# sebrahimi1988/dss-ml-at-scale

Hardware: NVIDIA H100
Metric: series fitted+forecast/sec (higher is better)
Workload: dtype f32

## Files before the change

dss-ml-at-scale_b200/csrc/fit_tc.cu:

```cuda
#include "mmf_internal.cuh"
#include "sm90_ptx.cuh"

namespace mmf {
namespace {

using namespace sm90;

constexpr int TILE_M = 128;
constexpr int KC = 32;
constexpr int NGROUPS = 2;
constexpr int FOLD_CHUNKS = 18;
constexpr int MAX_PRED = 64;
constexpr int BULK_MAX_PRED = 28;
constexpr int Y_STAGE_BYTES = TILE_M * KC * 4;
constexpr int AT_STAGE_BYTES = 2 * P * KC * 4;
constexpr int THREADS = 416;
constexpr int TILE_RING = 4;
constexpr int WARP_EPI0 = 8, WARP_PROD = 12;

template <int STAGES, int OBUF, bool SE = false>
struct SmemLayoutT {
  static constexpr int y = 0;
  static constexpr int at = y + STAGES * Y_STAGE_BYTES;
  static constexpr int apred = at + STAGES * AT_STAGE_BYTES;
  static constexpr int ostage = apred + MAX_PRED * P * 4;
  static constexpr int acc = ostage + OBUF * TILE_M * BULK_MAX_PRED * 4;
  static constexpr int nm = acc + 2 * NGROUPS * TILE_M * P * 4;
  static constexpr int cc = nm + 2 * NGROUPS * TILE_M * 2;
  static constexpr int tiles = cc + 2 * TILE_M * 4;
  static constexpr int bars = tiles + TILE_RING * 4;
  static constexpr int n_bars = 2 * STAGES + 6 + 2 * TILE_RING;
  static constexpr int ss = bars + n_bars * 8;
  static constexpr int sfac = ss + (SE ? 2 * NGROUPS * TILE_M * 8 : 0);
  static constexpr int total = sfac + (SE ? MAX_PRED * 4 : 0);
  static_assert(total + 1024 <= 232448, "exceeds the 227 KB of shared memory a CTA can opt into");
};

__device__ __forceinline__ float dot16(const float* __restrict__ arow, const float (&g)[P], float s) {
  const float4* ap = reinterpret_cast<const float4*>(arow);
  const float4 a0 = ap[0], a1 = ap[1], a2 = ap[2], a3 = ap[3];
  s = fmaf(a0.x, g[0], s);  s = fmaf(a0.y, g[1], s);  s = fmaf(a0.z, g[2], s);  s = fmaf(a0.w, g[3], s);
  s = fmaf(a1.x, g[4], s);  s = fmaf(a1.y, g[5], s);  s = fmaf(a1.z, g[6], s);  s = fmaf(a1.w, g[7], s);
  s = fmaf(a2.x, g[8], s);  s = fmaf(a2.y, g[9], s);  s = fmaf(a2.z, g[10], s); s = fmaf(a2.w, g[11], s);
  s = fmaf(a3.x, g[12], s); s = fmaf(a3.y, g[13], s); s = fmaf(a3.z, g[14], s); s = fmaf(a3.w, g[15], s);
  return s;
}

__device__ __forceinline__ bool is_finite_bits(float x) { return (__float_as_uint(x) & 0x7f800000u) != 0x7f800000u; }

__device__ __forceinline__ float centring_constant(const float4& a, const float4& b, int t_fit) {
  const float v[8] = {a.x, a.y, a.z, a.w, b.x, b.y, b.z, b.w};
  float c = t_fit > 7 ? v[7] : __int_as_float(0x7fc00000);
#pragma unroll
  for (int i = 6; i >= 0; --i) c = (i < t_fit && is_finite_bits(v[i])) ? v[i] : c;
  return c;
}

__device__ __forceinline__ void bt_write_moments(const BtArgs& bt, int k, int grp, int64_t n, const TileRec& tr, int frow0,
                                                 int t4, const float (&acc)[2][P], bool folded, const float* sacc) {
#pragma unroll
  for (int h = 0; h < 2; ++h)
#pragma unroll
    for (int j = 0; j < 2; ++j) {
      const int rt = 64 * h + frow0 + 8 * j;
      if (rt >= tr.nrows) continue;
      float* __restrict__ dst = bt.mom + (((int64_t)k * 2 + grp) * n + tr.row0 + rt) * P + 2 * t4;
#pragma unroll
      for (int i = 0; i < 2; ++i) {
        const int q = 4 * i + 2 * j;
        float2 v = make_float2(acc[h][q] + acc[h][q + P / 2], acc[h][q + 1] + acc[h][q + 1 + P / 2]);
        if (folded) {
          const float2 o = *reinterpret_cast<const float2*>(sacc + rt * P + 8 * i + 2 * t4);
          v.x = o.x + v.x; v.y = o.y + v.y;
        }
        *reinterpret_cast<float2*>(dst + 8 * i) = v;
      }
    }
}

__device__ __forceinline__ float lds32(uint32_t addr) {
  float v;
  asm volatile("ld.shared.f32 %0, [%1];" : "=f"(v) : "r"(addr));
  return v;
}

template <int STAGES, int OBUF, bool MULTI, bool SE = false, bool BT = false>
__global__ void __launch_bounds__(THREADS, 1)
fit_tc_kernel(const __grid_constant__ TcLaunch tl, const DesignView d, const FitArgs a,
              uint32_t* __restrict__ pending_count, const int n_tiles, const int n_chunks, const MultiView mv,
              const SeArgs se, const BtArgs bt) {
  static_assert(!SE || !MULTI, "standard errors are built for the single-calendar launch");
  static_assert(!BT || !(MULTI || SE), "backtests are built for the single-calendar launch");
  using SmemLayout = SmemLayoutT<STAGES, OBUF, SE>;
  auto tile_rec = [&](int ti) -> TileRec {
    if (MULTI) {
      if (ti >= n_tiles) return TileRec{0, 0, 0, 1};
      const int4 v = __ldg(reinterpret_cast<const int4*>(mv.tiles) + ti);
      return TileRec{v.x, v.y, v.z, v.w};
    }
    const int64_t left = a.n - (int64_t)ti * TILE_M;
    return TileRec{ti * TILE_M, (int)(left >= TILE_M ? TILE_M : (left > 0 ? left : 0)), 0, n_chunks};
  };
  extern __shared__ unsigned char smem_dyn[];
  unsigned char* smem = reinterpret_cast<unsigned char*>((reinterpret_cast<uintptr_t>(smem_dyn) + 1023) & ~uintptr_t(1023));
  const uint32_t sbase = smem_u32(smem);
  const uint32_t s_y = sbase + SmemLayout::y;
  const uint32_t s_at = sbase + SmemLayout::at;
  float* s_apred = reinterpret_cast<float*>(smem + SmemLayout::apred);
  float* s_ostage = reinterpret_cast<float*>(smem + SmemLayout::ostage);
  float* s_acc = reinterpret_cast<float*>(smem + SmemLayout::acc);
  uint16_t* s_nm = reinterpret_cast<uint16_t*>(smem + SmemLayout::nm);
  float* s_cc = reinterpret_cast<float*>(smem + SmemLayout::cc);
  double* s_ss = reinterpret_cast<double*>(smem + SmemLayout::ss);
  float* s_sfac = reinterpret_cast<float*>(smem + SmemLayout::sfac);
#ifdef MMF_TC_NO_COLLECT
  const bool collect = false;
#else
  const bool collect = a.recs != nullptr && d.t_fit <= 65535;
#endif
  const uint32_t s_bars = sbase + SmemLayout::bars;
  const int warp = threadIdx.x >> 5;
  const int lane = threadIdx.x & 31;
  auto bar_full = [&](int s) { return s_bars + 8u * s; };
  auto bar_empty = [&](int s) { return s_bars + 8u * (STAGES + s); };
  auto bar_accfull = [&](int b) { return s_bars + 8u * (2 * STAGES + b); };
  auto bar_accempty = [&](int b) { return s_bars + 8u * (2 * STAGES + 2 + b); };
  auto bar_cc = [&](int b) { return s_bars + 8u * (2 * STAGES + 4 + b); };
  auto bar_tfull = [&](int s) { return s_bars + 8u * (2 * STAGES + 6 + s); };
  auto bar_tempty = [&](int s) { return s_bars + 8u * (2 * STAGES + 6 + TILE_RING + s); };
  int* s_tiles = reinterpret_cast<int*>(smem + SmemLayout::tiles);
  auto take_tile = [&](int lt) -> int {
    const int sl = lt % TILE_RING;
    mbar_wait(bar_tfull(sl), (lt / TILE_RING) & 1);
    const int t = *reinterpret_cast<volatile int*>(s_tiles + sl);
    __syncwarp();
    if (lane == 0) mbar_arrive(bar_tempty(sl));
    return t;
  };

  if (blockIdx.x == 0 && threadIdx.x == 0 && a.zero_next != nullptr) {
#pragma unroll
    for (int i = 0; i < CTR_WORDS; ++i) a.zero_next[i] = 0u;
  }
  if (warp == WARP_PROD) {
    if (lane == 0) {
      for (int s = 0; s < STAGES; ++s) {
        mbar_init(bar_full(s), 1);
        mbar_init(bar_empty(s), 4);
      }
      for (int b = 0; b < 2; ++b) {
        mbar_init(bar_accfull(b), NGROUPS * 128);
        mbar_init(bar_accempty(b), 4);
        mbar_init(bar_cc(b), 128);
      }
      for (int sl = 0; sl < TILE_RING; ++sl) {
        mbar_init(bar_tfull(sl), 1);
        mbar_init(bar_tempty(sl), NGROUPS * 4 + 4);
      }
      fence_mbar_init();
      prefetch_tensormap(tl.tmap_y);
      prefetch_tensormap(tl.tmap_at);
    }
  } else if (warp >= WARP_EPI0) {
    if (!a.skip_pred && !MULTI)
      for (int i = threadIdx.x - WARP_EPI0 * 32; i < a.n_pred * P; i += 128)
        s_apred[i] = __ldg(d.apred + (size_t)a.pred_start * P + i);
    if (SE && !a.skip_pred)
      for (int i = threadIdx.x - WARP_EPI0 * 32; i < a.n_pred; i += 128) s_sfac[i] = __ldg(se.sfac + a.pred_start + i);
  }
  __syncthreads();
  if (threadIdx.x == 0) pdl_launch_dependents();

  if (warp == WARP_PROD) {
    int stage = 0;
    uint32_t phase = 0;
    int last_cal = -1;
    uint32_t* claim_ctr = pending_count + CTR_TILE_CLAIM;
    int tile = blockIdx.x;
    for (int lt = 0;; ++lt) {
      const int sl = lt % TILE_RING;
      mbar_wait(bar_tempty(sl), ((lt / TILE_RING) & 1) ^ 1u);
      const bool more = tile < n_tiles;
      uint32_t claim = 0;
      if (lane == 0) {
        if (more) claim = atomicAdd(claim_ctr, 1u);
        s_tiles[sl] = more ? tile : -1;
        mbar_arrive(bar_tfull(sl));
      }
      __syncwarp();
      if (!more) break;
      const TileRec tr = tile_rec(tile);
      const void* tmy = MULTI ? static_cast<const void*>(mv.tmaps_y + (size_t)tr.cal * 128) : static_cast<const void*>(tl.tmap_y);
      if (MULTI && tr.cal != last_cal) { fence_tensormap_acquire(tmy); last_cal = tr.cal; }
      const int at_row = MULTI ? tr.cal * 2 * P : 0;
      for (int ch = 0; ch < tr.n_chunks; ++ch) {
        mbar_wait(bar_empty(stage), phase ^ 1u);
        tma_load_2d_x2_elect(bar_full(stage), Y_STAGE_BYTES + AT_STAGE_BYTES,
                             s_y + stage * Y_STAGE_BYTES, tmy, ch * KC, tr.row0, L2_EVICT_NORMAL,
                             s_at + stage * AT_STAGE_BYTES, tl.tmap_at, ch * KC, at_row,
                             MULTI ? L2_EVICT_NORMAL : L2_EVICT_LAST);
        if (++stage == STAGES) { stage = 0; phase ^= 1u; }
      }
      tile = static_cast<int>(gridDim.x + __shfl_sync(0xffffffffu, claim, 0));
    }
  } else if (warp < NGROUPS * 4) {
    const int grp = warp >> 2;
    const int r = threadIdx.x & 127;
    const uint32_t row_off = static_cast<uint32_t>(r) * 128u;
    const uint32_t sw = static_cast<uint32_t>(r & 7);
    const int g8 = lane >> 2, t4 = lane & 3;
    const int frow0 = 16 * (warp & 3) + g8;
    uint32_t gc = 0;
    for (int lt = 0;; ++lt) {
      const int tile = take_tile(lt);
      if (tile < 0) break;
      const TileRec tr = tile_rec(tile);
      bool bad = false;
      float cf[2][2];
      float acc[2][P];
#pragma unroll
      for (int h = 0; h < 2; ++h)
#pragma unroll
        for (int i = 0; i < P; ++i) acc[h][i] = 0.f;
      const bool scan = collect && (!MULTI || r < tr.nrows);
      const int seg = (grp ^ (int)gc) & 1;
      int nm = 0;
      unsigned long long packq = 0ull;
      const int ab = lt & 1;
      float* __restrict__ sacc = s_acc + (ab * NGROUPS + grp) * TILE_M * P;
      auto sacc_at = [&](int h, int j, int i) {
        return reinterpret_cast<float2*>(sacc + (64 * h + frow0 + 8 * j) * P + 8 * i + 2 * t4);
      };
      bool folded = false;
      int since_fold = 0;
      double ssq[2][2] = {{0.0, 0.0}, {0.0, 0.0}};
      for (int ch = seg; ch < tr.n_chunks; ch += NGROUPS) {
        const uint32_t k = gc + static_cast<uint32_t>(ch);
        const int stage = static_cast<int>(k % STAGES);
        mbar_wait(bar_full(stage), (k / STAGES) & 1u);
        const uint32_t sy = s_y + stage * Y_STAGE_BYTES;
        if (ch == seg) {
          if (seg == 0) {
            mbar_wait(bar_accempty(ab), ((lt >> 1) & 1) ^ 1u);
            float c = 0.f;
            if (d.has_constant && r < tr.nrows) {
              const uint32_t rowp = sy + row_off;
              c = centring_constant(lds128(rowp + (sw << 4)), lds128(rowp + ((1u ^ sw) << 4)), MULTI ? KC : d.t_fit);
            }
            bad = collect && !is_finite_bits(c);
            s_cc[ab * TILE_M + r] = bad ? 0.f : c;
            mbar_arrive(bar_cc(ab));
          }
          mbar_wait(bar_cc(ab), (lt >> 1) & 1);
#pragma unroll
          for (int h = 0; h < 2; ++h)
#pragma unroll
            for (int j = 0; j < 2; ++j) cf[h][j] = s_cc[ab * TILE_M + 64 * h + frow0 + 8 * j];
        }
        if (scan) {
          const uint32_t rowp = sy + row_off;
          float4 v[8];
#pragma unroll
          for (int q = 0; q < 8; ++q) v[q] = lds128(rowp + ((static_cast<uint32_t>(q) ^ sw) << 4));
          float chk = 0.f;
#pragma unroll
          for (int q = 0; q < 8; ++q) {
            chk = fmaf(v[q].x, 0.f, chk); chk = fmaf(v[q].y, 0.f, chk);
            chk = fmaf(v[q].z, 0.f, chk); chk = fmaf(v[q].w, 0.f, chk);
          }
          if (!(chk == 0.f)) {
            unsigned gaps = 0u;
#pragma unroll
            for (int q = 0; q < 8; ++q)
              gaps |= (is_finite_bits(v[q].x) ? 0u : 1u << (4 * q)) | (is_finite_bits(v[q].y) ? 0u : 2u << (4 * q)) |
                      (is_finite_bits(v[q].z) ? 0u : 4u << (4 * q)) | (is_finite_bits(v[q].w) ? 0u : 8u << (4 * q));
            uint16_t* __restrict__ mt = a.recs[(int64_t)tr.row0 + r].miss_t + seg * SOLVE_SEG;
            const int tbase = ch * KC;
            while (gaps) {
              const int pos = __ffs(gaps) - 1;
              gaps &= gaps - 1u;
              packq = (packq >> 16) | (static_cast<unsigned long long>(tbase + pos) << 48);
              ++nm;
              if ((nm & 3) == 0 && nm <= SOLVE_SEG) *reinterpret_cast<unsigned long long*>(mt + nm - 4) = packq;
              if constexpr (BT) if (nm == SOLVE_SEG + 1)
                reinterpret_cast<uint16_t*>(&a.recs[(int64_t)tr.row0 + r].ss)[seg] = static_cast<uint16_t>(tbase + pos);
            }
          }
        }
        uint32_t ahi[2][KC / 8][4], alo[2][KC / 8][4];
        const int lim = d.t_fit - ch * KC;
#pragma unroll
        for (int h = 0; h < 2; ++h)
#pragma unroll
          for (int j = 0; j < 2; ++j) {
            const uint32_t rowp = sy + static_cast<uint32_t>(64 * h + frow0 + 8 * j) * 128u + t4 * 4;
            float part = 0.f;
#pragma unroll
            for (int kk = 0; kk < KC / 8; ++kk)
#pragma unroll
              for (int hf = 0; hf < 2; ++hf) {
                float x = lds32(rowp + ((static_cast<uint32_t>(2 * kk + hf) ^ static_cast<uint32_t>(g8)) << 4));
                if (collect) x = is_finite_bits(x) ? x : cf[h][j];
                const float rr = x - cf[h][j];
                const uint32_t hb = __float_as_uint(rr) & 0xFFFFE000u;
                ahi[h][kk][j + 2 * hf] = hb;
                alo[h][kk][j + 2 * hf] = __float_as_uint(rr - __uint_as_float(hb));
                if (SE) {
                  const float rs = 4 * (2 * kk + hf) + t4 < lim ? rr : 0.f;
                  part = fmaf(rs, rs, part);
                }
              }
            if (SE) ssq[h][j] += static_cast<double>(part);
          }
        const uint64_t bdesc0 = gmma_desc_k_sw128(s_at + stage * AT_STAGE_BYTES);
        uint32_t bt_in = 0;
        if constexpr (BT) {
          const int s0 = ch * KC;
          uint32_t pre = 0;
#pragma unroll
          for (int k = 0; k < MMF_BT_MAX_ORIGINS - 1; ++k) {
            pre |= (bt.t_orig[k] >= s0 - KC && bt.t_orig[k] <= s0 ? 1u : 0u) << k;
            bt_in |= (bt.t_orig[k] > s0 && bt.t_orig[k] < s0 + KC ? 1u : 0u) << k;
          }
          while (pre) {
            const int k = __ffs(pre) - 1;
            pre &= pre - 1u;
            bt_write_moments(bt, k, grp, a.n, tr, frow0, t4, acc, folded, sacc);
          }
        }
        if constexpr (BT) {
        if (bt_in != 0u) {
          int lo = 0;
          uint32_t m = bt_in;
          for (;;) {
            const int k = m ? __ffs(m) - 1 : -1;
            const int hi = k >= 0 ? __ldg(&bt.cals[k].t_fit) - ch * KC : KC;
            wgmma_fence();
#pragma unroll
            for (int h = 0; h < 2; ++h)
#pragma unroll
              for (int kk = 0; kk < KC / 8; ++kk) {
                const uint64_t bdesc = bdesc0 + static_cast<uint64_t>(kk * 2);
                uint32_t fh[4], fl[4];
#pragma unroll
                for (int e = 0; e < 4; ++e) {
                  const int col = 8 * kk + 4 * (e >> 1) + t4;
                  const bool in = col >= lo && col < hi;
                  fh[e] = in ? ahi[h][kk][e] : 0u;
                  fl[e] = in ? alo[h][kk][e] : 0u;
                }
                wgmma_m64n32k8_tf32_rs(acc[h], fh, bdesc);
#ifndef MMF_TC_NO_LO_TERM
                wgmma_m64n32k8_tf32_rs(acc[h], fl, bdesc);
#endif
              }
            wgmma_commit();
            wgmma_wait<0>();
            wgmma_fence_regs(acc[0]);
            wgmma_fence_regs(acc[1]);
            if (k < 0) break;
            bt_write_moments(bt, k, grp, a.n, tr, frow0, t4, acc, folded, sacc);
            m &= m - 1u;
            lo = hi;
          }
        } else {
        wgmma_fence();
#pragma unroll
        for (int h = 0; h < 2; ++h)
#pragma unroll
          for (int kk = 0; kk < KC / 8; ++kk) {
            const uint64_t bdesc = bdesc0 + static_cast<uint64_t>(kk * 2);
            wgmma_m64n32k8_tf32_rs(acc[h], ahi[h][kk], bdesc);
#ifndef MMF_TC_NO_LO_TERM
            wgmma_m64n32k8_tf32_rs(acc[h], alo[h][kk], bdesc);
#endif
          }
        wgmma_commit();
        wgmma_wait<0>();
        wgmma_fence_regs(acc[0]);
        wgmma_fence_regs(acc[1]);
        }
        } else {
        wgmma_fence();
#pragma unroll
        for (int h = 0; h < 2; ++h)
#pragma unroll
          for (int kk = 0; kk < KC / 8; ++kk) {
            const uint64_t bdesc = bdesc0 + static_cast<uint64_t>(kk * 2);
            wgmma_m64n32k8_tf32_rs(acc[h], ahi[h][kk], bdesc);
#ifndef MMF_TC_NO_LO_TERM
            wgmma_m64n32k8_tf32_rs(acc[h], alo[h][kk], bdesc);
#endif
          }
        wgmma_commit();
        wgmma_wait<0>();
        wgmma_fence_regs(acc[0]);
        wgmma_fence_regs(acc[1]);
        }
        __syncwarp();
        if (lane == 0) mbar_arrive(bar_empty(stage));
        if (++since_fold == FOLD_CHUNKS && ch + NGROUPS < tr.n_chunks) {
          if (!folded) mbar_wait(bar_accempty(ab), ((lt >> 1) & 1) ^ 1u);
#pragma unroll
          for (int h = 0; h < 2; ++h)
#pragma unroll
            for (int j = 0; j < 2; ++j)
#pragma unroll
              for (int i = 0; i < 2; ++i) {
                const int q = 4 * i + 2 * j;
                float2 f = make_float2(acc[h][q] + acc[h][q + P / 2], acc[h][q + 1] + acc[h][q + 1 + P / 2]);
                if (folded) { const float2 o = *sacc_at(h, j, i); f.x = o.x + f.x; f.y = o.y + f.y; }
                *sacc_at(h, j, i) = f;
              }
#pragma unroll
          for (int h = 0; h < 2; ++h)
#pragma unroll
            for (int i = 0; i < P; ++i) acc[h][i] = 0.f;
          folded = true;
          since_fold = 0;
        }
      }
      if (scan && (nm & 3) != 0 && nm < SOLVE_SEG) {
        uint16_t* __restrict__ mt = a.recs[(int64_t)tr.row0 + r].miss_t + seg * SOLVE_SEG;
        *reinterpret_cast<unsigned long long*>(mt + (nm & ~3)) = packq >> (16 * (4 - (nm & 3)));
      }
      if constexpr (BT) {
        const int s_end = ((tr.n_chunks - 1 - seg) / NGROUPS * NGROUPS + seg + 1) * KC;
        uint32_t rest = 0;
#pragma unroll
        for (int k = 0; k < MMF_BT_MAX_ORIGINS - 1; ++k) rest |= (bt.t_orig[k] != INT32_MAX && bt.t_orig[k] >= s_end ? 1u : 0u) << k;
        while (rest) {
          const int k = __ffs(rest) - 1;
          rest &= rest - 1u;
          bt_write_moments(bt, k, grp, a.n, tr, frow0, t4, acc, folded, sacc);
        }
      }
      if (!folded) mbar_wait(bar_accempty(ab), ((lt >> 1) & 1) ^ 1u);
#pragma unroll
      for (int h = 0; h < 2; ++h)
#pragma unroll
        for (int j = 0; j < 2; ++j)
#pragma unroll
          for (int i = 0; i < 2; ++i) {
            const int q = 4 * i + 2 * j;
            float2 v = make_float2(acc[h][q] + acc[h][q + P / 2], acc[h][q + 1] + acc[h][q + 1 + P / 2]);
            if (folded) { const float2 o = *sacc_at(h, j, i); v.x = o.x + v.x; v.y = o.y + v.y; }
            *sacc_at(h, j, i) = v;
          }
      if (SE) {
#pragma unroll
        for (int h = 0; h < 2; ++h)
#pragma unroll
          for (int j = 0; j < 2; ++j) {
            double v = ssq[h][j];
            v += __shfl_xor_sync(0xffffffffu, v, 1);
            v += __shfl_xor_sync(0xffffffffu, v, 2);
            if (t4 == 0) s_ss[(ab * NGROUPS + grp) * TILE_M + 64 * h + frow0 + 8 * j] = v;
          }
      }
      const int cnt = nm > 0x7ffe ? 0x7ffe : nm;
      s_nm[(ab * NGROUPS + seg) * TILE_M + r] = static_cast<uint16_t>(cnt | (bad ? 0x8000 : 0));
      mbar_arrive(bar_accfull(ab));
      gc += static_cast<uint32_t>(tr.n_chunks);
    }
  } else {
    const int r = threadIdx.x & 127;
    bool vec_out = (a.n_pred % 4 == 0) && (a.ld_out % 4 == 0) && ((reinterpret_cast<uintptr_t>(a.out) & 15u) == 0);
    for (int i = 0; i + 1 < a.n_out; ++i) vec_out = vec_out && ((reinterpret_cast<uintptr_t>(a.out_more[i]) & 15u) == 0);
#ifdef MMF_TC_NO_BULK
    const bool bulk = false;
#else
    const bool bulk = !a.skip_pred && vec_out && a.out_multimem != 1 && a.ld_out == a.n_pred && a.n_pred <= BULK_MAX_PRED;
#endif
    const uint32_t s_ostage_u32 = smem_u32(s_ostage);
    const uint64_t l2_policy = l2_evict_first_policy();
    const bool se_vec = SE && (a.n_pred % 4 == 0) && (se.ld_se % 4 == 0) &&
                        ((reinterpret_cast<uintptr_t>(se.out_se) & 15u) == 0);
    int lt = 0;
    int cur_cal = MULTI ? -1 : 0;
    uint32_t kept_mask = d.kept_mask;
    int t_fit_c = d.t_fit;
    for (;; ++lt) {
      const int tile = take_tile(lt);
      if (tile < 0) break;
      const int ab = lt & 1;
      const TileRec tr = tile_rec(tile);
      const int64_t row = (int64_t)tr.row0 + r;
      const bool live = r < tr.nrows;
      if (MULTI && tr.cal != cur_cal) {
        const int4* cp = reinterpret_cast<const int4*>(mv.cals + tr.cal);
        const int4 m0 = __ldg(cp), m1 = __ldg(cp + 1);
        t_fit_c = m0.x;
        kept_mask = static_cast<uint32_t>(m0.w);
        if (!a.skip_pred) {
          named_bar_sync(2, 128);
          const float* __restrict__ src = d.apred + (size_t)(m1.x + m1.y) * P;
          for (int i = threadIdx.x - WARP_EPI0 * 32; i < a.n_pred * P; i += 128) s_apred[i] = __ldg(src + i);
          named_bar_sync(2, 128);
        }
        cur_cal = tr.cal;
      }
      mbar_wait(bar_accfull(ab), (lt >> 1) & 1);
      float c = s_cc[ab * TILE_M + r];
      float g[P];
      {
        const float4* p0 = reinterpret_cast<const float4*>(s_acc + (ab * NGROUPS + 0) * TILE_M * P + r * P);
        const float4* p1 = reinterpret_cast<const float4*>(s_acc + (ab * NGROUPS + 1) * TILE_M * P + r * P);
#pragma unroll
        for (int q = 0; q < P / 4; ++q) {
          const float4 u = p0[q], w = p1[q];
          g[4 * q] = u.x + w.x; g[4 * q + 1] = u.y + w.y; g[4 * q + 2] = u.z + w.z; g[4 * q + 3] = u.w + w.w;
        }
      }
      const unsigned f0 = s_nm[(ab * NGROUPS + 0) * TILE_M + r], f1 = s_nm[(ab * NGROUPS + 1) * TILE_M + r];
      const double ss = SE ? s_ss[(ab * NGROUPS + 0) * TILE_M + r] + s_ss[(ab * NGROUPS + 1) * TILE_M + r] : 0.0;
      if constexpr (BT) {
        __syncwarp();
        if (lane == 0) mbar_arrive(bar_accempty(ab));
        for (int k = 0; k < bt.n_origin; ++k) {
          const bool last = k == bt.n_origin - 1;
          const int4 m0 = __ldg(reinterpret_cast<const int4*>(bt.cals + k));
          const int tk = m0.x;
          float gk[P];
          if (last || !live) {
#pragma unroll
            for (int p = 0; p < P; ++p) gk[p] = g[p];
          } else {
            const float4* p0 = reinterpret_cast<const float4*>(bt.mom + (((int64_t)k * NGROUPS + 0) * a.n + row) * P);
            const float4* p1 = reinterpret_cast<const float4*>(bt.mom + (((int64_t)k * NGROUPS + 1) * a.n + row) * P);
#pragma unroll
            for (int q = 0; q < P / 4; ++q) {
              const float4 u = p0[q], w = p1[q];
              gk[4 * q] = u.x + w.x; gk[4 * q + 1] = u.y + w.y; gk[4 * q + 2] = u.z + w.z; gk[4 * q + 3] = u.w + w.w;
            }
          }
          const SolveRec* __restrict__ src = collect ? a.recs + row : nullptr;
          int n0 = f0 & 0x7fff, n1 = f1 & 0x7fff;
          bool over = false;
          if (collect && !last && live && (n0 | n1) != 0) {
#pragma unroll
            for (int sg = 0; sg < 2; ++sg) {
              const int tot = sg ? n1 : n0;
              const uint16_t* mt = src->miss_t + sg * SOLVE_SEG;
              const int have = tot < SOLVE_SEG ? tot : SOLVE_SEG;
              int cnt = 0;
              while (cnt < have && mt[cnt] < tk) ++cnt;
              if (cnt == SOLVE_SEG && tot > SOLVE_SEG && reinterpret_cast<const uint16_t*>(&src->ss)[sg] < tk) over = true;
              if (sg) n1 = cnt; else n0 = cnt;
            }
          }
          bool general = false;
          if (collect)
            general = ((f0 | f1) & 0x8000u) != 0u || over || n0 > SOLVE_SEG || n1 > SOLVE_SEG || 2 * (n0 + n1) > tk;
          bool finite = true;
#pragma unroll
          for (int p = 0; p < P; ++p) {
            finite = finite && is_finite_bits(gk[p]);
            if (!((kept_mask >> p) & 1u)) gk[p] = 0.f;
          }
          const bool pend = live && (!finite || general);
          const bool defer = live && !pend && (n0 + n1) > 0;
          const unsigned pm = __ballot_sync(0xffffffffu, pend);
          if (lane == 0 && pm != 0u) {
            atomicAdd(pending_count, __popc(pm));
            atomicAdd(bt.pending + k, __popc(pm));
          }
          const unsigned dm = __ballot_sync(0xffffffffu, defer);
          if (dm != 0u) {
            unsigned base = 0;
            if (lane == 0) base = atomicAdd(bt.rec_count + k, __popc(dm));
            base = __shfl_sync(0xffffffffu, base, 0);
            if (defer) {
              SolveRec& rec = bt.recs[(int64_t)k * a.n + row];
              float bk[P];
              if (last) {
#pragma unroll
                for (int p = 0; p < P; ++p) bk[p] = gk[p];
              } else {
                const float* __restrict__ tm = bt.tmat + (size_t)k * P * P;
#pragma unroll
                for (int p = 0; p < P; ++p) {
                  float s = 0.f;
#pragma unroll
                  for (int q = 0; q < P; ++q) s = fmaf(__ldg(tm + q * P + p), gk[q], s);
                  bk[p] = s;
                }
                for (int sg = 0; sg < 2; ++sg) {
                  const int cnt = sg ? n1 : n0;
                  for (int e = 0; e < cnt; ++e) rec.miss_t[sg * SOLVE_SEG + e] = src->miss_t[sg * SOLVE_SEG + e];
                }
              }
              float4* bp = reinterpret_cast<float4*>(rec.b);
              bp[0] = make_float4(bk[0], bk[1], bk[2], bk[3]);    bp[1] = make_float4(bk[4], bk[5], bk[6], bk[7]);
              bp[2] = make_float4(bk[8], bk[9], bk[10], bk[11]);  bp[3] = make_float4(bk[12], bk[13], bk[14], bk[15]);
              rec.c = c;
              rec.nm[0] = static_cast<uint16_t>(n0);
              rec.nm[1] = static_cast<uint16_t>(n1);
              rec.cal = k;
              const unsigned slot = base + __popc(dm & ((1u << lane) - 1u));
              if (slot < a.rec_cap) bt.rec_rows[(int64_t)k * a.n + slot] = row;
            }
          }
          if (live && !pend && !defer) {
            const float* __restrict__ pk = bt.pred + (size_t)k * a.n_pred * P;
            const int64_t off = ((int64_t)k * bt.out_kstride + row) * a.ld_out;
            if (vec_out) {
              for (int j = 0; j < a.n_pred; j += 4) {
                float o[4];
#pragma unroll
                for (int w = 0; w < 4; ++w) o[w] = dot16(pk + (j + w) * P, gk, c);
                store_out4(a, off + j, make_float4(o[0], o[1], o[2], o[3]));
              }
            } else {
              for (int j = 0; j < a.n_pred; ++j) store_out1(a, off + j, dot16(pk + j * P, gk, c));
            }
          }
          if (live) a.status[(int64_t)k * bt.st_kstride + row] = pend ? MMF_STATUS_PENDING : (defer ? MMF_STATUS_DEFERRED : MMF_STATUS_OK);
        }
        continue;
      }
      __syncwarp();
      if (lane == 0) mbar_arrive(bar_accempty(ab));
      int nm0 = 0, nm1 = 0;
      bool general = false;
      if (collect) {
        nm0 = f0 & 0x7fff; nm1 = f1 & 0x7fff;
        general = ((f0 | f1) & 0x8000u) != 0u || nm0 > SOLVE_SEG || nm1 > SOLVE_SEG || 2 * (nm0 + nm1) > t_fit_c;
        if (general) c = 0.f;
      }
      bool finite = true;
#pragma unroll
      for (int p = 0; p < P; ++p) {
        finite = finite && is_finite_bits(g[p]);
        if (!((kept_mask >> p) & 1u)) g[p] = 0.f;
      }
      const bool pend = live && (!finite || general);
      const bool defer = live && !pend && (nm0 + nm1) > 0;
      const unsigned pm = __ballot_sync(0xffffffffu, pend);
      if (lane == 0 && pm != 0u) {
        atomicAdd(pending_count, __popc(pm));
        if (MULTI) atomicAdd(mv.pending_by_cal + tr.cal, __popc(pm));
      }
      const unsigned dm = __ballot_sync(0xffffffffu, defer);
      if (dm != 0u) {
        unsigned base = 0;
        if (lane == 0) base = atomicAdd(a.rec_count, __popc(dm));
        base = __shfl_sync(0xffffffffu, base, 0);
        if (defer) {
          SolveRec& rec = a.recs[row];
          float4* bp = reinterpret_cast<float4*>(rec.b);
          bp[0] = make_float4(g[0], g[1], g[2], g[3]);    bp[1] = make_float4(g[4], g[5], g[6], g[7]);
          bp[2] = make_float4(g[8], g[9], g[10], g[11]);  bp[3] = make_float4(g[12], g[13], g[14], g[15]);
          rec.c = c;
          if (SE) rec.ss = static_cast<float>(ss);
          rec.nm[0] = static_cast<uint16_t>(nm0);
          rec.nm[1] = static_cast<uint16_t>(nm1);
          rec.cal = tr.cal;
          const unsigned slot = base + __popc(dm & ((1u << lane) - 1u));
          if (slot < a.rec_cap) a.rec_rows[slot] = row;
        }
      }
      if (bulk) {
        const int ob = OBUF > 1 ? (lt % OBUF) : 0;
        if (warp == WARP_EPI0) { if (OBUF > 1) bulk_wait_read1_elect(); else bulk_wait_read_elect(); }
        named_bar_sync(1, 128);
        float* __restrict__ srow = s_ostage + ob * (TILE_M * BULK_MAX_PRED) + r * a.n_pred;
        for (int k = 0; k < a.n_pred; k += 4) {
          float o[4];
#pragma unroll
          for (int w = 0; w < 4; ++w) o[w] = dot16(s_apred + (k + w) * P, g, c);
          *reinterpret_cast<float4*>(srow + k) = make_float4(o[0], o[1], o[2], o[3]);
        }
        fence_proxy_async_smem();
        named_bar_sync(1, 128);
        const uint32_t bytes = static_cast<uint32_t>(tr.nrows) * a.n_pred * 4u;
        const int64_t off = (int64_t)tr.row0 * a.n_pred;
        const uint32_t src = s_ostage_u32 + static_cast<uint32_t>(ob) * (TILE_M * BULK_MAX_PRED * 4);
        for (uint32_t i = r; i < bytes / 16u; i += 128u)
          stg128_hint(reinterpret_cast<float4*>(a.out + off) + i, lds128(src + 16u * i), l2_policy);
        if (warp == WARP_EPI0) {
          const int n_peer = a.n_out - 1;
          int j = n_peer > 1 ? tile % n_peer : 0;
          for (int i = 0; i < n_peer; ++i) {
            bulk_store_elect(reinterpret_cast<uint64_t>(a.out_more[j] + off), src, bytes);
            if (++j == n_peer) j = 0;
          }
          bulk_commit_elect();
        }
      } else if (live && !pend && !defer && !a.skip_pred) {
        const int64_t off = row * a.ld_out;
        if (vec_out) {
          for (int k = 0; k < a.n_pred; k += 4) {
            float o[4];
#pragma unroll
            for (int w = 0; w < 4; ++w) o[w] = dot16(s_apred + (k + w) * P, g, c);
            store_out4(a, off + k, make_float4(o[0], o[1], o[2], o[3]));
          }
        } else {
          for (int k = 0; k < a.n_pred; ++k) store_out1(a, off + k, dot16(s_apred + k * P, g, c));
        }
      }
      if (live) {
        if (!pend && !defer) {
          if (a.out_gamma != nullptr) {
            float4* gp = reinterpret_cast<float4*>(a.out_gamma + row * P);
            gp[0] = make_float4(g[0], g[1], g[2], g[3]);    gp[1] = make_float4(g[4], g[5], g[6], g[7]);
            gp[2] = make_float4(g[8], g[9], g[10], g[11]);  gp[3] = make_float4(g[12], g[13], g[14], g[15]);
            a.out_c[row] = c;
          }
          if (a.out_beta != nullptr) {
            float* __restrict__ br = a.out_beta + row * P;
            for (int p = 0; p < P; ++p) {
              float s = (p == 0 && d.has_constant) ? c : 0.f;
#pragma unroll
              for (int q = 0; q < P; ++q) s = fmaf(__ldg(d.w + p * P + q), g[q], s);
              br[p] = s;
            }
          }
          if (SE) {
            double bg = 0.0;
#pragma unroll
            for (int p = 0; p < P; ++p) bg = fma(static_cast<double>(g[p]), static_cast<double>(g[p]), bg);
            const int dof = t_fit_c - __popc(kept_mask);
            const double rss = fmax(ss - bg, 0.0);
            const float sig = dof > 0 ? static_cast<float>(sqrt(rss / dof)) : __int_as_float(0x7fc00000);
            se.sigma[row] = sig;
            if (se.dof != nullptr) se.dof[row] = dof;
            if (se.out_se != nullptr && !a.skip_pred) {
              float* __restrict__ srow = se.out_se + row * se.ld_se;
              int k = 0;
              if (se_vec)
                for (; k < a.n_pred; k += 4)
                  __stcs(reinterpret_cast<float4*>(srow + k),
                         make_float4(sig * s_sfac[k], sig * s_sfac[k + 1], sig * s_sfac[k + 2], sig * s_sfac[k + 3]));
              for (; k < a.n_pred; ++k) __stcs(srow + k, sig * s_sfac[k]);
            }
          }
        }
        stg32_hint(a.status + row, pend ? MMF_STATUS_PENDING : (defer ? MMF_STATUS_DEFERRED : MMF_STATUS_OK), l2_policy);
      }
    }
    if (bulk && warp == WARP_EPI0) bulk_wait_all_elect();
  }
}

}

bool fit_tc_supported(const DesignView& d, const FitArgs& a, const char** why) {
  const char* w = nullptr;
  if (!a.skip_pred && a.n_pred > MAX_PRED) w = "n_pred > 64 needs the fit + predict_tc_kernel pair";
  else if (a.n_pred < 1) w = "n_pred < 1";
  else if (a.ld_y % 4 != 0) w = "ld_y not a multiple of 4 floats (TMA needs 16-B row pitch)";
  else if ((reinterpret_cast<uintptr_t>(a.y) & 15u) != 0) w = "y not 16-B aligned";
  else if (d.t_fit < 1) w = "t_fit < 1";
  else if (a.n > (int64_t)0x7fffffff - TILE_M) w = "n too large for 32-bit TMA coordinates";
  if (why) *why = w;
  return w == nullptr;
}

template <int STAGES, int OBUF, bool MULTI, bool SE = false, bool BT = false>
static cudaError_t launch_variant(const DesignView& d, const FitArgs& a, const TcLaunch& tl, uint32_t* pending_count,
                                  int sm_count, cudaStream_t s, int n_tiles, int n_chunks, const MultiView& mv,
                                  const SeArgs& se = SeArgs{}, const BtArgs& bt = BtArgs{}) {
  const size_t smem = SmemLayoutT<STAGES, OBUF, SE>::total + 1024;
  cudaError_t e = cudaFuncSetAttribute(fit_tc_kernel<STAGES, OBUF, MULTI, SE, BT>, cudaFuncAttributeMaxDynamicSharedMemorySize, (int)smem);
  if (e != cudaSuccess) return e;
  const int grid = n_tiles < sm_count ? n_tiles : sm_count;
  fit_tc_kernel<STAGES, OBUF, MULTI, SE, BT><<<grid, THREADS, smem, s>>>(tl, d, a, pending_count, n_tiles, n_chunks, mv, se, bt);
  return cudaGetLastError();
}

cudaError_t launch_fit_tc(const DesignView& d, const FitArgs& a, const TcLaunch& tl, uint32_t* pending_count,
                          int sm_count, cudaStream_t s, int variant, const MultiView* multi) {
  if (a.n <= 0) return cudaSuccess;
  if (multi != nullptr)
    return launch_variant<8, 1, true>(d, a, tl, pending_count, sm_count, s, multi->n_tiles, 2, *multi);
  const int n_tiles = (int)((a.n + TILE_M - 1) / TILE_M);
  const int n_chunks = d.t_pad / KC;
  const MultiView none{};
  return variant == 2 ? launch_variant<6, 2, false>(d, a, tl, pending_count, sm_count, s, n_tiles, n_chunks, none)
                      : launch_variant<8, 1, false>(d, a, tl, pending_count, sm_count, s, n_tiles, n_chunks, none);
}

cudaError_t launch_fit_tc_se(const DesignView& d, const FitArgs& a, const TcLaunch& tl, uint32_t* pending_count,
                             int sm_count, cudaStream_t s, const SeArgs& se) {
  if (a.n <= 0) return cudaSuccess;
  const int n_tiles = (int)((a.n + TILE_M - 1) / TILE_M);
  return launch_variant<8, 1, false, true>(d, a, tl, pending_count, sm_count, s, n_tiles, d.t_pad / KC, MultiView{}, se);
}

cudaError_t launch_fit_tc_bt(const DesignView& d, const FitArgs& a, const TcLaunch& tl, uint32_t* pending_count,
                             int sm_count, cudaStream_t s, const BtArgs& bt) {
  if (a.n <= 0) return cudaSuccess;
  const int n_tiles = (int)((a.n + TILE_M - 1) / TILE_M);
  return launch_variant<8, 1, false, false, true>(d, a, tl, pending_count, sm_count, s, n_tiles, d.t_pad / KC,
                                                  MultiView{}, SeArgs{}, bt);
}

}
```

Baseline: 634.8 million.

## Claim runs of four contiguous tiles and store forecasts as one contiguous block

Adds a RUN template mode where the producer claims runs of consecutive tiles with one atomic. The epilogue stages each tile's forecasts into its own slot of a four-slot output buffer, and the whole run is written to global memory as one contiguous span. The aim is fewer atomic claims and fewer, larger global stores per run. In exchange the pipeline drops from 8 to 6 stages to make room for the larger staging buffer, and the tail runs get coarser, which can unbalance load across SMs.

Result: faster. 646.7 million (median of 6 runs) (+1.9%).

```diff
diff --git a/dss-ml-at-scale_b200/csrc/fit_tc.cu b/dss-ml-at-scale_b200/csrc/fit_tc.cu
--- a/dss-ml-at-scale_b200/csrc/fit_tc.cu
+++ b/dss-ml-at-scale_b200/csrc/fit_tc.cu
@@ -16,6 +16,7 @@
 constexpr int AT_STAGE_BYTES = 2 * P * KC * 4;
 constexpr int THREADS = 416;
 constexpr int TILE_RING = 4;
+constexpr int RUN_CONT = 1 << 30;
 constexpr int WARP_EPI0 = 8, WARP_PROD = 12;
 
 template <int STAGES, int OBUF, bool SE = false>
@@ -46,6 +47,19 @@
   return s;
 }
 
+__host__ __device__ __forceinline__ bool staged_table(const FitArgs& a) {
+#ifdef MMF_TC_NO_BULK
+  return false;
+#else
+  return !a.skip_pred && a.n_pred % 4 == 0 && a.ld_out == a.n_pred && a.n_pred <= BULK_MAX_PRED &&
+         (reinterpret_cast<uintptr_t>(a.out) & 15u) == 0 && a.out_multimem != 1;
+#endif
+}
+
+__host__ __device__ __forceinline__ bool run_claims(const FitArgs& a, int n_tiles, int grid, int run) {
+  return run > 1 && staged_table(a) && a.n_out == 1 && a.out_multimem == 0 && n_tiles >= 2 * run * grid;
+}
+
 __device__ __forceinline__ bool is_finite_bits(float x) { return (__float_as_uint(x) & 0x7f800000u) != 0x7f800000u; }
 
 __device__ __forceinline__ float centring_constant(const float4& a, const float4& b, int t_fit) {
@@ -84,13 +98,14 @@
   return v;
 }
 
-template <int STAGES, int OBUF, bool MULTI, bool SE = false, bool BT = false>
+template <int STAGES, int OBUF, bool MULTI, bool SE = false, bool BT = false, int RUN = 1>
 __global__ void __launch_bounds__(THREADS, 1)
 fit_tc_kernel(const __grid_constant__ TcLaunch tl, const DesignView d, const FitArgs a,
               uint32_t* __restrict__ pending_count, const int n_tiles, const int n_chunks, const MultiView mv,
               const SeArgs se, const BtArgs bt) {
   static_assert(!SE || !MULTI, "standard errors are built for the single-calendar launch");
   static_assert(!BT || !(MULTI || SE), "backtests are built for the single-calendar launch");
+  static_assert(RUN == 1 || (!MULTI && !BT && OBUF == RUN), "runs stage one tile per staging slot, single calendar");
   using SmemLayout = SmemLayoutT<STAGES, OBUF, SE>;
   auto tile_rec = [&](int ti) -> TileRec {
     if (MULTI) {
@@ -176,15 +191,19 @@
     uint32_t phase = 0;
     int last_cal = -1;
     uint32_t* claim_ctr = pending_count + CTR_TILE_CLAIM;
-    int tile = blockIdx.x;
+    const int run = RUN > 1 && run_claims(a, n_tiles, static_cast<int>(gridDim.x), RUN) ? RUN : 1;
+    int tile = static_cast<int>(blockIdx.x) * run;
+    int run_end = tile + run < n_tiles ? tile + run : n_tiles;
     for (int lt = 0;; ++lt) {
       const int sl = lt % TILE_RING;
       mbar_wait(bar_tempty(sl), ((lt / TILE_RING) & 1) ^ 1u);
       const bool more = tile < n_tiles;
-      uint32_t claim = 0;
+      const bool ends = RUN == 1 || tile + 1 >= run_end;
+      uint32_t claim = 0, size = 1;
       if (lane == 0) {
-        if (more) claim = atomicAdd(claim_ctr, 1u);
-        s_tiles[sl] = more ? tile : -1;
+        if (RUN > 1 && n_tiles - tile > 2 * run * static_cast<int>(gridDim.x)) size = static_cast<uint32_t>(run);
+        if (more && ends) claim = atomicAdd(claim_ctr, RUN > 1 ? size : 1u);
+        s_tiles[sl] = more ? (tile | (ends ? 0 : RUN_CONT)) : -1;
         mbar_arrive(bar_tfull(sl));
       }
       __syncwarp();
@@ -201,7 +220,15 @@
                              MULTI ? L2_EVICT_NORMAL : L2_EVICT_LAST);
         if (++stage == STAGES) { stage = 0; phase ^= 1u; }
       }
-      tile = static_cast<int>(gridDim.x + __shfl_sync(0xffffffffu, claim, 0));
+      if (RUN > 1 && !ends) {
+        ++tile;
+      } else {
+        tile = static_cast<int>(static_cast<uint32_t>(run) * gridDim.x + __shfl_sync(0xffffffffu, claim, 0));
+        if (RUN > 1) {
+          const int len = static_cast<int>(__shfl_sync(0xffffffffu, size, 0));
+          run_end = tile + len < n_tiles ? tile + len : n_tiles;
+        }
+      }
     }
   } else if (warp < NGROUPS * 4) {
     const int grp = warp >> 2;
@@ -212,8 +239,9 @@
     const int frow0 = 16 * (warp & 3) + g8;
     uint32_t gc = 0;
     for (int lt = 0;; ++lt) {
-      const int tile = take_tile(lt);
+      int tile = take_tile(lt);
       if (tile < 0) break;
+      if (RUN > 1) tile &= ~RUN_CONT;
       const TileRec tr = tile_rec(tile);
       bool bad = false;
       float cf[2][2];
@@ -480,9 +508,13 @@
     int cur_cal = MULTI ? -1 : 0;
     uint32_t kept_mask = d.kept_mask;
     int t_fit_c = d.t_fit;
+    int run_pos = 0;
+    int64_t run_row0 = 0;
     for (;; ++lt) {
-      const int tile = take_tile(lt);
+      int tile = take_tile(lt);
       if (tile < 0) break;
+      const bool ends_run = RUN == 1 || (tile & RUN_CONT) == 0;
+      if (RUN > 1) tile &= ~RUN_CONT;
       const int ab = lt & 1;
       const TileRec tr = tile_rec(tile);
       const int64_t row = (int64_t)tr.row0 + r;
@@ -661,23 +693,30 @@
         }
       }
       if (bulk) {
-        const int ob = OBUF > 1 ? (lt % OBUF) : 0;
-        if (warp == WARP_EPI0) { if (OBUF > 1) bulk_wait_read1_elect(); else bulk_wait_read_elect(); }
-        named_bar_sync(1, 128);
-        float* __restrict__ srow = s_ostage + ob * (TILE_M * BULK_MAX_PRED) + r * a.n_pred;
+        const int ob = RUN > 1 ? run_pos : (OBUF > 1 ? (lt % OBUF) : 0);
+        if (RUN == 1 || run_pos == 0) {
+          if (warp == WARP_EPI0) { if (OBUF > 1 && RUN == 1) bulk_wait_read1_elect(); else bulk_wait_read_elect(); }
+          named_bar_sync(1, 128);
+          if (RUN > 1) run_row0 = tr.row0;
+        }
+        float* __restrict__ srow = s_ostage + (ob * TILE_M + r) * a.n_pred;
         for (int k = 0; k < a.n_pred; k += 4) {
           float o[4];
 #pragma unroll
           for (int w = 0; w < 4; ++w) o[w] = dot16(s_apred + (k + w) * P, g, c);
           *reinterpret_cast<float4*>(srow + k) = make_float4(o[0], o[1], o[2], o[3]);
         }
+        if (ends_run) {
         fence_proxy_async_smem();
         named_bar_sync(1, 128);
         const uint32_t bytes = static_cast<uint32_t>(tr.nrows) * a.n_pred * 4u;
         const int64_t off = (int64_t)tr.row0 * a.n_pred;
-        const uint32_t src = s_ostage_u32 + static_cast<uint32_t>(ob) * (TILE_M * BULK_MAX_PRED * 4);
-        for (uint32_t i = r; i < bytes / 16u; i += 128u)
-          stg128_hint(reinterpret_cast<float4*>(a.out + off) + i, lds128(src + 16u * i), l2_policy);
+        const uint32_t src = s_ostage_u32 + static_cast<uint32_t>(ob * TILE_M * a.n_pred * 4);
+        const uint32_t run_bytes = RUN > 1 ? bytes + static_cast<uint32_t>(run_pos * TILE_M * a.n_pred * 4) : bytes;
+        const int64_t run_off = RUN > 1 ? run_row0 * a.n_pred : off;
+        const uint32_t run_src = RUN > 1 ? s_ostage_u32 : src;
+        for (uint32_t i = r; i < run_bytes / 16u; i += 128u)
+          stg128_hint(reinterpret_cast<float4*>(a.out + run_off) + i, lds128(run_src + 16u * i), l2_policy);
         if (warp == WARP_EPI0) {
           const int n_peer = a.n_out - 1;
           int j = n_peer > 1 ? tile % n_peer : 0;
@@ -687,6 +726,8 @@
           }
           bulk_commit_elect();
         }
+        }
+        if (RUN > 1) run_pos = ends_run ? 0 : run_pos + 1;
       } else if (live && !pend && !defer && !a.skip_pred) {
         const int64_t off = row * a.ld_out;
         if (vec_out) {
@@ -758,15 +799,17 @@
   return w == nullptr;
 }
 
-template <int STAGES, int OBUF, bool MULTI, bool SE = false, bool BT = false>
+template <int STAGES, int OBUF, bool MULTI, bool SE = false, bool BT = false, int RUN = 1>
 static cudaError_t launch_variant(const DesignView& d, const FitArgs& a, const TcLaunch& tl, uint32_t* pending_count,
                                   int sm_count, cudaStream_t s, int n_tiles, int n_chunks, const MultiView& mv,
                                   const SeArgs& se = SeArgs{}, const BtArgs& bt = BtArgs{}) {
   const size_t smem = SmemLayoutT<STAGES, OBUF, SE>::total + 1024;
-  cudaError_t e = cudaFuncSetAttribute(fit_tc_kernel<STAGES, OBUF, MULTI, SE, BT>, cudaFuncAttributeMaxDynamicSharedMemorySize, (int)smem);
+  cudaError_t e = cudaFuncSetAttribute(fit_tc_kernel<STAGES, OBUF, MULTI, SE, BT, RUN>,
+                                       cudaFuncAttributeMaxDynamicSharedMemorySize, (int)smem);
   if (e != cudaSuccess) return e;
   const int grid = n_tiles < sm_count ? n_tiles : sm_count;
-  fit_tc_kernel<STAGES, OBUF, MULTI, SE, BT><<<grid, THREADS, smem, s>>>(tl, d, a, pending_count, n_tiles, n_chunks, mv, se, bt);
+  fit_tc_kernel<STAGES, OBUF, MULTI, SE, BT, RUN>
+      <<<grid, THREADS, smem, s>>>(tl, d, a, pending_count, n_tiles, n_chunks, mv, se, bt);
   return cudaGetLastError();
 }
 
@@ -778,8 +821,11 @@
   const int n_tiles = (int)((a.n + TILE_M - 1) / TILE_M);
   const int n_chunks = d.t_pad / KC;
   const MultiView none{};
-  return variant == 2 ? launch_variant<6, 2, false>(d, a, tl, pending_count, sm_count, s, n_tiles, n_chunks, none)
-                      : launch_variant<8, 1, false>(d, a, tl, pending_count, sm_count, s, n_tiles, n_chunks, none);
+  if (variant == 2) return launch_variant<6, 2, false>(d, a, tl, pending_count, sm_count, s, n_tiles, n_chunks, none);
+  const int grid = n_tiles < sm_count ? n_tiles : sm_count;
+  if (run_claims(a, n_tiles, grid, 4))
+    return launch_variant<6, 4, false, false, false, 4>(d, a, tl, pending_count, sm_count, s, n_tiles, n_chunks, none);
+  return launch_variant<8, 1, false>(d, a, tl, pending_count, sm_count, s, n_tiles, n_chunks, none);
 }
 
 cudaError_t launch_fit_tc_se(const DesignView& d, const FitArgs& a, const TcLaunch& tl, uint32_t* pending_count,
```
